# Anony-CFFM/CFFM

Measured on AMD Instinct MI355X. Metric: training examples/sec, frappe 10-field dim32; embedding-gather %HBM roofline, higher is better.
Workload: dtype f32; 1 GPU; frappe shape: synthetic libfm, 10 fields, 5382 features, inner/outer dim 32, batch 256 per GPU, selu, Adagrad lr 0.05, square_loss (README.md:28); global_batch=256, id_distribution=uniform, tables=replicated, parallelism=single

## Files before the change

### cffm_amd/csrc/common.hpp

```cpp
#pragma once
#include <hip/hip_runtime.h>
#include <stdint.h>

#include "../../include/cffm_hip.h"

#define CFFM_WAVE 64

#ifdef CFFM_PHASE_TIMERS
static __device__ unsigned long long cffm_phase_times[16];
static __device__ unsigned long long cffm_wg_times[2 * 1024];
static __device__ unsigned long long cffm_bwd_times[48];
#define PHASE_MARKB(i, wg) do { if ((wg) == 7 && threadIdx.x == 0) cffm_bwd_times[i] = wall_clock64(); } while (0)
#define PHASE_MARK(i) do { if (blockIdx.x == 7 && threadIdx.x == 0) cffm_phase_times[i] = wall_clock64(); } while (0)
#define PHASE_MARK2(i) do {} while (0)
#define PHASE_MARK3(i) do { if (CL && blockIdx.x == 7 && threadIdx.x == 0) cffm_phase_times[8 + (i)] = wall_clock64(); } while (0)
#else
#define PHASE_MARK(i) do {} while (0)
#define PHASE_MARK2(i) do {} while (0)
#define PHASE_MARK3(i) do {} while (0)
#define PHASE_MARKB(i, wg) do {} while (0)
#endif

typedef float f32x4 __attribute__((ext_vector_type(4)));
__device__ __forceinline__ int fused_c_off(int l, int c0, int c1, int D, int Pp) {
// ... 180 lines not shown
static inline int conv_slabs(const cffm_shape_t* s, int32_t B, int l) {
    const int64_t S = s->D >> (l + 1);
    if (bwd_fused01_ok(s, B)) {
        if (l <= 1) return 256;
        const int64_t n = ((int64_t)B * S * S + CFFM_TOP_SLAB_ROWS - 1) / CFFM_TOP_SLAB_ROWS;
        return n < 1 ? 1 : (int)n;
    }
    if (bwd_top_ok(s, B) && l >= bwd_top_first_layer(s)) {
        if (!top_wgrad_deferred(s, B)) return 256;
        const int64_t n = ((int64_t)B * S * S + 63) / 64;
        return n < 1 ? 1 : (n > 256 ? 256 : (int)n);
    }
    return conv_slabs_plain(s, B, l);
}

static inline void make_slab_plan(const cffm_shape_t* s, int32_t B, const cffm_theta_layout_t& tl, SlabPlan* p) {
    int n = 0;
    int64_t base = 0;
    auto add = [&](int64_t off, int64_t end, int nslab) {
        p->r[n].off = off; p->r[n].len = end - off; p->r[n].base = base; p->r[n].nslab = nslab;
        base += (end - off) * nslab;
        return n++;
    };
    const int64_t convs = tl.live > 0 ? tl.conv_w[0] : tl.d1_w;
    p->head_front = add(0, tl.inner_cw, small_slabs(B));
    p->inner = add(tl.inner_cw, convs, small_slabs(B));
    p->conv0 = n;
    for (int l = 0; l < tl.live; ++l)
        add(tl.conv_w[l], l + 1 < tl.live ? tl.conv_w[l + 1] : tl.d1_w, conv_slabs(s, B, l));
    p->head_back = add(tl.d1_w, tl.n, small_slabs(B));
    p->n = n;
    p->total = base;
}

__device__ __forceinline__ float head_dout(int loss, float out, float y, float invB, float L) {
    switch (loss) {
        case CFFM_LOSS_SQUARE_RMSE: return (out - y) * invB / L;
        case CFFM_LOSS_MSE: return 2.f * (out - y) * invB;
        case CFFM_LOSS_MAE: return (out > y ? 1.f : (out < y ? -1.f : 0.f)) * invB;
        case CFFM_LOSS_SQUARE_L2: return out - y;
        case CFFM_LOSS_HYBRID:
            return 0.5f * (out - y) - 0.5f * invB * (y / (out + 1e-7f) - (1.f - y) / (1.f - out + 1e-7f));
        default: {
            const float s = out;
            return -(y / (s + 1e-7f) - (1.f - y) / (1.f - s + 1e-7f)) * invB * s * (1.f - s);
        }
    }
}

#define CFFM_SELU_SCALE 1.0507009873554804934193349852946f
#define CFFM_SELU_SCALE_ALPHA 1.7580993408473768599402175208123f

__device__ __forceinline__ float act_f(float x, int act) {
    switch (act) {
        case CFFM_ACT_RELU: return fmaxf(x, 0.f);
        case CFFM_ACT_PRELU: return fmaxf(x, 0.f) + 0.25f * (-fmaxf(-x, 0.f));
        case CFFM_ACT_ELU: return x < 0.f ? expf(x) - 1.f : x;
        case CFFM_ACT_SELU: return x < 0.f ? CFFM_SELU_SCALE_ALPHA * (expf(x) - 1.f) : CFFM_SELU_SCALE * x;
        default: return x * (0.5f * (1.f + erff(x * 0.70710678118654752440f)));
    }
}

__device__ __forceinline__ float act_grad_f(float x, int act) {
    switch (act) {
        case CFFM_ACT_RELU: return x > 0.f ? 1.f : 0.f;
        case CFFM_ACT_PRELU: return x > 0.f ? 1.f : (x < 0.f ? 0.25f : 0.f);
        case CFFM_ACT_ELU: return x < 0.f ? expf(x) : 1.f;
        case CFFM_ACT_SELU: return x < 0.f ? CFFM_SELU_SCALE_ALPHA * expf(x) : CFFM_SELU_SCALE;
        default: {
            float cdf = 0.5f * (1.f + erff(x * 0.70710678118654752440f));
            float pdf = expf(-0.5f * x * x) * 0.39894228040143267794f;
            return cdf + x * pdf;
        }
    }
}

__device__ __forceinline__ float act_pos(float c, int act) {
    switch (act) {
        case CFFM_ACT_SELU: return CFFM_SELU_SCALE * c;
        case CFFM_ACT_GELU: return c * (0.5f * (1.f + erff(c * 0.70710678118654752440f)));
        default: return c;
    }
}

__device__ __forceinline__ float act_relu_grad(float c, int act) {
    return c > 0.f ? act_grad_f(c, act) : 0.f;
}

__device__ __forceinline__ void lds_barrier() {
    __builtin_amdgcn_fence(__ATOMIC_RELEASE, "workgroup", "local");
    __builtin_amdgcn_s_barrier();
    __builtin_amdgcn_fence(__ATOMIC_ACQUIRE, "workgroup", "local");
}

template <int CTRL, int ROW_MASK>
__device__ __forceinline__ float dpp_mov(float v, float identity) {
    return __builtin_bit_cast(float, __builtin_amdgcn_update_dpp(__builtin_bit_cast(int, identity), __builtin_bit_cast(int, v),
                                                                 CTRL, ROW_MASK, 0xf, false));
}
__device__ __forceinline__ float wave_sum(float v) {
    v += dpp_mov<0xB1, 0xf>(v, 0.f);
    v += dpp_mov<0x4E, 0xf>(v, 0.f);
    v += dpp_mov<0x141, 0xf>(v, 0.f);
    v += dpp_mov<0x140, 0xf>(v, 0.f);
    v += dpp_mov<0x142, 0xa>(v, 0.f);
    v += dpp_mov<0x143, 0xc>(v, 0.f);
    return __builtin_bit_cast(float, __builtin_amdgcn_readlane(__builtin_bit_cast(int, v), 63));
}
__device__ __forceinline__ float wave_max(float v) {
    const float ninf = -INFINITY;
    v = fmaxf(v, dpp_mov<0xB1, 0xf>(v, ninf));
    v = fmaxf(v, dpp_mov<0x4E, 0xf>(v, ninf));
    v = fmaxf(v, dpp_mov<0x141, 0xf>(v, ninf));
    v = fmaxf(v, dpp_mov<0x140, 0xf>(v, ninf));
    v = fmaxf(v, dpp_mov<0x142, 0xa>(v, ninf));
    v = fmaxf(v, dpp_mov<0x143, 0xc>(v, ninf));
    return __builtin_bit_cast(float, __builtin_amdgcn_readlane(__builtin_bit_cast(int, v), 63));
}

template <bool SIXTEEN>
__device__ __forceinline__ float row_group_sum(float v) {
    v += dpp_mov<0xB1, 0xf>(v, 0.f);
    v += dpp_mov<0x4E, 0xf>(v, 0.f);
    v += dpp_mov<0x141, 0xf>(v, 0.f);
    if (SIXTEEN) v += dpp_mov<0x140, 0xf>(v, 0.f);
    return v;
}

template <int NTH = 0>
__device__ __forceinline__ float block_sum(float v, float* red) {
    v = wave_sum(v);
    const int w = threadIdx.x >> 6, nw = NTH ? NTH >> 6 : (int)blockDim.x >> 6;
    __syncthreads();
    if ((threadIdx.x & 63) == 0 && (NTH == 0 || w < nw)) red[w] = v;
    __syncthreads();
    float t = 0.f;
    for (int i = 0; i < nw; ++i) t += red[i];
    return t;
}

template <int NTH = 0>
__device__ __forceinline__ void build_pair_lut(uint32_t* lut, int F, int Pp) {
    const int nth = NTH ? NTH : (int)blockDim.x;
    for (int i = threadIdx.x; i < F; i += nth) {
        int base = i * (2 * F - i - 1) / 2;
        for (int j = i + 1; j < F; ++j) lut[base + j - i - 1] = (uint32_t)i | ((uint32_t)j << 16);
    }
    const int P = F * (F - 1) / 2;
    for (int p = P + threadIdx.x; p < Pp; p += nth) lut[p] = 0u;
}

__device__ __forceinline__ int fast_div(int n, float inv_d) { return (int)(((float)n + 0.5f) * inv_d); }

__device__ __forceinline__ f32x4 mfma16(float a, float b, f32x4 c) {
    return __builtin_amdgcn_mfma_f32_16x16x4f32(a, b, c, 0, 0, 0);
}


template <int N, int NTH>
struct ParkFilter {
    float4 w[N];
    float4* dst;
    int n4;
    __device__ __forceinline__ void fetch(const float4* src, float4* dst_, int n4_) {
        dst = dst_; n4 = src != nullptr ? n4_ : 0;
#pragma unroll
        for (int ii = 0; ii < N; ++ii) {
            const int i = threadIdx.x + NTH * ii;
            w[ii] = i < n4 ? src[i] : make_float4(0.f, 0.f, 0.f, 0.f);
        }
    }
    __device__ __forceinline__ void operator()() const {
#pragma unroll
        for (int ii = 0; ii < N; ++ii) {
            const int i = threadIdx.x + NTH * ii;
            if (i < n4) dst[i] = w[ii];
        }
    }
};

template <int U, int NTH, class T, class Load, class Use>
__device__ __forceinline__ void loads_first(int tid, int n, Load&& load, Use&& use) {
    for (int e0 = tid; e0 < n; e0 += U * NTH) {
        T v[U];
#pragma unroll
        for (int u = 0; u < U; ++u) {
            const int e = e0 + u * NTH;
            if (e < n) v[u] = load(e);
        }
#pragma unroll
        for (int u = 0; u < U; ++u) {
            const int e = e0 + u * NTH;
            if (e < n) use(e, v[u]);
        }
    }
}
```

### cffm_amd/csrc/conv.hip

```cpp
#include <cstdlib>
#include <cstring>

#include "internal.hpp"

#include <type_traits>

#include <stdlib.h>
#include "inner_body.hpp"
#include "head_body.hpp"
#include "sort_body.hpp"

#define KSTEP 32
#define WG_KM 64

__device__ __forceinline__ int64_t xcd_tile(int64_t per_xcd) {
    const int64_t id = blockIdx.x;
    return (id & 7) * per_xcd + (id >> 3);
}
__host__ __device__ static inline int64_t xcd_per(int64_t tiles) { return (tiles + 7) / 8; }

struct RowPos { int b, y, x; };
__device__ __forceinline__ RowPos row_pos(int64_t m, int lgSo) {
    RowPos p;
    const int So = 1 << lgSo;
// ... 1549 lines not shown
    unsigned long long* keys_sorted;
    int live, n_rows, id_bits, B;
    int rank_keys;
    int c0_off, c1_off;
    int early_off, es_off;
};


__device__ __forceinline__ unsigned rank_key_id(int raw, int M) { return min((unsigned)raw, (unsigned)M); }
template <int NW, int F_ = 0>
__device__ __forceinline__ void rank_keys_body(const int32_t* __restrict__ ids, int n, int b, int F_rt, int M,
                                               unsigned long long* __restrict__ out, char* smem) {
    constexpr int MAXF = F_ ? F_ : RANK_MAXF;
    const int F = F_ ? F_ : F_rt;
    float* cnt = reinterpret_cast<float*>(smem);
    const int tid = threadIdx.x, lane = tid & 63, wave = tid >> 6;
    unsigned long long mine[MAXF];
#pragma unroll
    for (int f = 0; f < MAXF; ++f) {
        const int slot = b * F + (f < F ? f : 0);
        mine[f] = f < F ? (((unsigned long long)rank_key_id(ids[slot], M) << 32) | (unsigned)slot) : 0ull;
    }
    int c[MAXF];
#pragma unroll
    for (int f = 0; f < MAXF; ++f) c[f] = 0;
    constexpr int GRP = 8;
    for (int j0 = tid; j0 < n; j0 += 64 * NW * GRP) {
        unsigned idj[GRP];
#pragma unroll
        for (int u = 0; u < GRP; ++u) {
            const int j = j0 + 64 * NW * u;
            idj[u] = rank_key_id(ids[j < n ? j : n - 1], M);
        }
#pragma unroll
        for (int u = 0; u < GRP; ++u) {
            const int j = j0 + 64 * NW * u;
            const unsigned long long kj = j < n ? (((unsigned long long)idj[u] << 32) | (unsigned)j) : ~0ull;
#pragma unroll
            for (int f = 0; f < MAXF; ++f) c[f] += kj < mine[f] ? 1 : 0;
        }
    }
#pragma unroll
    for (int f = 0; f < MAXF; ++f) {
        const float t = wave_sum((float)c[f]);
        if (lane == 0) cnt[wave * RANK_MAXF + f] = t;
    }
    __syncthreads();
    if (tid < F) {
        float c = cnt[tid];
#pragma unroll
        for (int w = 1; w < NW; ++w) c += cnt[w * RANK_MAXF + tid];
        const int rank = (int)c;
        const int slot = b * F + tid;
        out[rank] = ((unsigned long long)rank_key_id(ids[slot], M) << 32) | (unsigned)slot;
    }
    __syncthreads();
}

template <int N> using IntC = std::integral_constant<int, N>;
#define CV(x) decltype(x)::value
template <int L0, int L1, class Fn>
__device__ __forceinline__ void static_for(Fn&& fn) {
    if constexpr (L0 < L1) { fn(IntC<L0>()); static_for<L0 + 1, L1>(fn); }
}

template <int NT, int G, int ACT, int LGSO = -1, int GT = G>
__device__ __forceinline__ void fused_layer_fwd(const ConvArgs& ca, int b, char* smem, const float* inL, float* outL) {
    const int lgSo = LGSO >= 0 ? LGSO : ca.lgSo;
    const int64_t rows = 1ll << (2 * lgSo), m_lo = (int64_t)b * rows, m_hi = m_lo + rows;
    if (rows >= 64) {
        for (int64_t m0 = m_lo; m0 < m_hi; m0 += 64) {
            if (m0 > m_lo) lds_barrier();
            conv_fwd_taps_body<NT, 4 / G, false, G, ACT, LGSO, GT>(ca, m0, m_hi, smem, inL, outL, m_lo);
        }
    } else if (rows >= 32) {
        conv_fwd_taps_body<NT, (G >= 2 ? 1 : 2), false, G, ACT, LGSO, GT>(ca, m_lo, m_hi, smem, inL, outL, m_lo);
    } else {
        conv_fwd_taps_body<NT, 1, false, G, ACT, LGSO, GT>(ca, m_lo, m_hi, smem, inL, outL, m_lo);
    }
}

static constexpr int fwd_all_layer_groups(int G, int lgSo) { return (G > 2 && lgSo <= 1) ? 2 : G; }

template <int NT, int NW, int ACT = -1, int F_ = 0, int K_ = 0, int D_ = 0>
__global__ __launch_bounds__(64 * NW) void fwd_all_kernel(FwdAllArgs fa) {
    constexpr int G = NW / 4, PP = NT * 16;
    constexpr bool CS = F_ != 0;
    constexpr FwdAllLds PL = fwd_all_lds_plan(CS ? F_ : 2, CS ? K_ : 4, CS ? D_ : 4, PP, NW);
    constexpr int NTS = CS ? 512 : 0;
    static_assert(!CS || 64 * NW >= NTS, "the workgroup holds the threads that sum inner_out");
    static_assert(!CS || (F_ * (F_ - 1) / 2 + 15) / 16 * 16 == PP, "NT is the column tile count of F_ fields");
    static_assert(!CS || (PL.c0_off >= 0 && PL.early_fits), "the compiled shape keeps its activations in LDS and gathers early");
    extern __shared__ __attribute__((aligned(16))) char smem[];
    const int c0_off = CS ? PL.c0_off : fa.c0_off, c1_off = CS ? PL.c1_off : fa.c1_off, es_off = CS ? PL.es_off : fa.es_off;
    const int D = CS ? D_ : fa.inner.g.D;
    int live = fa.live;
    if (CS) { live = -1; for (int d = D_; d > 1; d >>= 1) ++live; }
    auto CL = [&](int l) -> float* {
        return c0_off >= 0 ? reinterpret_cast<float*>(smem + fused_c_off(l, c0_off, c1_off, D, PP)) : nullptr;
    };
    const bool lds_act = c0_off >= 0;
#ifdef CFFM_PHASE_TIMERS
    if (threadIdx.x == 0) cffm_wg_times[2 * blockIdx.x] = wall_clock64();
#endif
    auto example = [&](int b) __attribute__((always_inline)) {
        ParkFilter<(4 * PP * PP / 4 + 64 * NW - 1) / (64 * NW), 64 * NW> park;
        const bool early = fa.early_off > 0;
        park.fetch(early ? reinterpret_cast<const float4*>(fa.conv[0].W) : nullptr, reinterpret_cast<float4*>(smem), 4 * PP * PP / 4);
        char* smem_i = smem + (CS ? (early ? PL.t_off : 0) : fa.early_off);
        if (fa.rank_keys) rank_keys_body<NW, F_>(fa.ids, fa.n_rows, b, fa.inner.g.F, fa.inner.g.M, fa.keys_sorted, smem_i);
        PHASE_MARK(0);
        inner_fwd_body<ACT, decltype(park), F_, K_, D_, NTS>(fa.inner, b, smem_i, early ? reinterpret_cast<float*>(smem + es_off) : nullptr,
                                                             D + 1, park);
        if (lds_act) lds_barrier(); else __syncthreads();
        PHASE_MARK(1);
        conv0_fact_fwd_body<NT, NW, F_, D_>(fa.conv[0], b, smem, CL(0), early);
        if constexpr (CS) {
            static_for<1, PL.live>([&](auto lc) __attribute__((always_inline)) {
                constexpr int l = CV(lc), LGSO = PL.lgS0 - l;
                lds_barrier();
                PHASE_MARK(1 + l);
                fused_layer_fwd<NT, fwd_all_layer_groups(G, LGSO), ACT, LGSO, G>(fa.conv[l], b, smem, CL(l - 1), CL(l));
            });
        } else {
            for (int l = 1; l < live; ++l) {
                if (lds_act) lds_barrier(); else __syncthreads();
                PHASE_MARK(1 + l);
                fused_layer_fwd<NT, G, ACT>(fa.conv[l], b, smem, CL(l - 1), CL(l));
            }
        }
        if (lds_act) lds_barrier(); else __syncthreads();
        PHASE_MARK(1 + live);
        head_fwd_body<NW, ACT, false, F_, D_>(fa.head, b, smem, lds_act, c0_off, c1_off);
        PHASE_MARK(2 + live);
    };
    if constexpr (CS) {
        static_assert(!CS || 4096 / (CS ? F_ : 1) <= 2 * 256, "two passes over a grid of 256 workgroups cover every accepted B");
        if ((int)blockIdx.x < fa.B) example((int)blockIdx.x);
        if (const int b = blockIdx.x + gridDim.x; b < fa.B) {
            __syncthreads();
            example(b);
        }
    } else {
        for (int b = blockIdx.x; b < fa.B; b += gridDim.x) {
            if (b != (int)blockIdx.x) __syncthreads();
            example(b);
        }
    }
#ifdef CFFM_PHASE_TIMERS
    if (threadIdx.x == 0) cffm_wg_times[2 * blockIdx.x + 1] = wall_clock64();
#endif
}

template <int NT, int F_, int D_, int NW, bool ONE = false>
__device__ __forceinline__ void conv0_fact_bwd_body(const DgradArgs& a, float* __restrict__ slabW, float* __restrict__ slabB,
                                                    int64_t slab_stride, char* smem, int wg, int nwg) {
    constexpr int PP = NT * 16, S = 16, NTH = 64 * NW, XQ = 16 / NW;
    const int F = F_ ? F_ : a.F, D = D_ ? D_ : a.D, Dp = D + 1, P = F_ ? F_ * (F_ - 1) / 2 : a.P, F2 = 2 * F;
    const int TP = S * PP + 16;
    float* Wl = reinterpret_cast<float*>(smem);
    float* T = Wl + 4 * PP * PP;
    float* part = T + 2 * F * TP;
    float* dEi = part + NW * 16 * 32;
    float* dEj = dEi + 32 * 16;
    float* bred = dEj + 32 * 16;
    float* rs = bred + NW * PP;
    float* Es = rs + 2 * F;
    const int tid = threadIdx.x, lane = tid & 63, wave = tid >> 6, r = lane & 15, kk = lane >> 4;
    float* sw = slabW + (int64_t)wg * slab_stride;
    float* sb = slabB + (int64_t)wg * slab_stride;
    PHASE_MARKB(12, wg);
    {
        ParkFilter<(4 * PP * PP / 4 + NTH - 1) / NTH, NTH> park;
        park.fetch(reinterpret_cast<const float4*>(a.W), reinterpret_cast<float4*>(Wl), 4 * PP * PP / 4);
        park();
        for (int e = tid; e < 4 * (PP - P) * PP; e += NTH) {
            const int tap = e / ((PP - P) * PP), o = e - tap * ((PP - P) * PP);
            sw[(tap * PP + P) * PP + o] = 0.f;
        }
    }
    bool first = true;
    float bacc[NT];
#pragma unroll
    for (int nt = 0; nt < NT; ++nt) bacc[nt] = 0.f;

    for (int b = wg; b < a.B; b += nwg) {
        __syncthreads();
        {
            const float* e = a.Cprev + (int64_t)b * F * D;
            const float invD = 1.f / (float)D;
            loads_first<2, NTH, float>(tid, F * D, [&](int i) { return e[i]; }, [&](int i, float v) {
                const int f = fast_div(i, invD), d = i - f * D;
                Es[f * Dp + d] = v;
            });
        }
        __syncthreads();
        const float* dCb = a.dC + (int64_t)b * S * S * PP;
        PHASE_MARKB(13, wg);
        for (int u = wave; u < 2 * (F - 1); u += NW) {
            const int i = u % (F - 1), dh = u / (F - 1);
            const int nj = F - 1 - i, K = 2 * nj, base = i * (2 * F - i - 1) / 2;
            f32x4 acc[NT];
#pragma unroll
            for (int nt = 0; nt < NT; ++nt) acc[nt] = (f32x4){0.f, 0.f, 0.f, 0.f};
            for (int k0 = 0; k0 < K; k0 += 4) {
                const int k = k0 + kk;
                const bool ok = k < K;
                const int dw = (ok && k >= nj) ? 1 : 0, jj = ok ? k - dw * nj : 0;
                const float av = ok ? Es[(i + 1 + jj) * Dp + 2 * r + dw] : 0.f;
                const float* wr = Wl + ((dh * 2 + dw) * PP + base + jj) * PP + r;
#pragma unroll
                for (int nt = 0; nt < NT; ++nt) acc[nt] = mfma16(av, ok ? wr[nt * 16] : 0.f, acc[nt]);
            }
            float* tp = T + (dh * F + i) * TP + r;
#pragma unroll
            for (int nt = 0; nt < NT; ++nt)
#pragma unroll
                for (int j = 0; j < 4; ++j) tp[(kk * 4 + j) * PP + nt * 16] = acc[nt][j];
        }
        for (int e = tid; e < 2 * S * PP; e += NTH) {
            const int dh = e / (S * PP), o = e - dh * (S * PP);
            T[(dh * F + F - 1) * TP + o] = 0.f;
        }
        __syncthreads();
        PHASE_MARKB(14, wg);
        {
            f32x4 acc[2] = {(f32x4){0.f, 0.f, 0.f, 0.f}, (f32x4){0.f, 0.f, 0.f, 0.f}};
            float4 av[XQ][NT];
#pragma unroll
            for (int q4 = 0; q4 < XQ; ++q4)
#pragma unroll
                for (int h = 0; h < NT; ++h)
                    av[q4][h] = *reinterpret_cast<const float4*>(dCb + ((int64_t)r * S + wave + NW * q4) * PP + 16 * h + 4 * kk);
#pragma unroll
            for (int q4 = 0; q4 < XQ; ++q4) {
                const int x = wave + NW * q4;
#pragma unroll
                for (int h = 0; h < NT; ++h) {
                    float4 bv[2];
#pragma unroll
                    for (int ct = 0; ct < 2; ++ct) {
                        const int n = ct * 16 + r;
                        bv[ct] = n < F2 ? *reinterpret_cast<const float4*>(T + n * TP + x * PP + 16 * h + 4 * kk)
                                        : make_float4(0.f, 0.f, 0.f, 0.f);
                    }
#pragma unroll
                    for (int ct = 0; ct < 2; ++ct) {
                        acc[ct] = mfma16(av[q4][h].x, bv[ct].x, acc[ct]);
                        acc[ct] = mfma16(av[q4][h].y, bv[ct].y, acc[ct]);
                        acc[ct] = mfma16(av[q4][h].z, bv[ct].z, acc[ct]);
                        acc[ct] = mfma16(av[q4][h].w, bv[ct].w, acc[ct]);
                    }
                }
            }
#pragma unroll
            for (int ct = 0; ct < 2; ++ct)
#pragma unroll
                for (int j = 0; j < 4; ++j) part[(wave * 16 + kk * 4 + j) * 32 + ct * 16 + r] = acc[ct][j];
        }
        __syncthreads();
        for (int e = tid; e < 16 * 32; e += NTH) {
            float v = part[e];
#pragma unroll
            for (int w = 1; w < NW; ++w) v += part[512 * w + e];
            dEi[(e & 31) * 16 + (e >> 5)] = v;
        }
        __syncthreads();
        PHASE_MARKB(15, wg);
        {
            float av[2][4];
#pragma unroll
            for (int rt = 0; rt < 2; ++rt)
#pragma unroll
                for (int s4 = 0; s4 < 4; ++s4) {
                    const int m = rt * 16 + r, dh = m >= F ? 1 : 0, i = m - dh * F;
                    av[rt][s4] = m < F2 ? Es[i * Dp + 2 * (4 * s4 + kk) + dh] : 0.f;
                }
#pragma unroll
            for (int q4 = 0; q4 < XQ; ++q4) {
                const int x = wave + NW * q4;
                float bv[4][NT];
#pragma unroll
                for (int s4 = 0; s4 < 4; ++s4)
#pragma unroll
                    for (int nt = 0; nt < NT; ++nt) bv[s4][nt] = dCb[((int64_t)(4 * s4 + kk) * S + x) * PP + nt * 16 + r];
                f32x4 acc[2][NT];
#pragma unroll
                for (int rt = 0; rt < 2; ++rt)
#pragma unroll
                    for (int nt = 0; nt < NT; ++nt) acc[rt][nt] = (f32x4){0.f, 0.f, 0.f, 0.f};
#pragma unroll
                for (int s4 = 0; s4 < 4; ++s4)
#pragma unroll
                    for (int nt = 0; nt < NT; ++nt) {
                        bacc[nt] += bv[s4][nt];
#pragma unroll
                        for (int rt = 0; rt < 2; ++rt) acc[rt][nt] = mfma16(av[rt][s4], bv[s4][nt], acc[rt][nt]);
                    }
#pragma unroll
                for (int rt = 0; rt < 2; ++rt)
#pragma unroll
                    for (int nt = 0; nt < NT; ++nt)
#pragma unroll
                        for (int j = 0; j < 4; ++j) {
                            const int m = rt * 16 + kk * 4 + j;
                            if (m < F2) T[m * TP + x * PP + nt * 16 + r] = acc[rt][nt][j];
                        }
            }
        }
        __syncthreads();
        PHASE_MARKB(16, wg);
        {
            int ucount = 0;
            for (int dh = 0; dh < 2; ++dh)
                for (int i = 0; i < F - 1; ++i) {
                    const int nj = F - 1 - i, K = 2 * nj, base = i * (2 * F - i - 1) / 2;
                    for (int rt = 0; rt * 16 < K; ++rt, ++ucount) {
                        if ((ucount & (NW - 1)) != wave) continue;
                        const int m = rt * 16 + r;
                        const bool okm = m < K;
                        const int dw = (okm && m >= nj) ? 1 : 0, jj = okm ? m - dw * nj : 0;
                        f32x4 acc[NT];
#pragma unroll
                        for (int nt = 0; nt < NT; ++nt) acc[nt] = (f32x4){0.f, 0.f, 0.f, 0.f};
#pragma unroll
                        for (int s4 = 0; s4 < 4; ++s4) {
                            const int x = 4 * s4 + kk;
                            const float avv = okm ? Es[(i + 1 + jj) * Dp + 2 * x + dw] : 0.f;
                            const float* tb = T + (dh * F + i) * TP + x * PP + r;
#pragma unroll
                            for (int nt = 0; nt < NT; ++nt) acc[nt] = mfma16(avv, tb[nt * 16], acc[nt]);
                        }
#pragma unroll
                        for (int j = 0; j < 4; ++j) {
                            const int mm = rt * 16 + kk * 4 + j;
                            if (mm < K) {
                                const int dw2 = mm >= nj ? 1 : 0, jj2 = mm - dw2 * nj;
                                float* dst = sw + ((dh * 2 + dw2) * PP + base + jj2) * PP + r;
#pragma unroll
                                for (int nt = 0; nt < NT; ++nt) dst[nt * 16] = first ? acc[nt][j] : dst[nt * 16] + acc[nt][j];
                            }
                        }
                    }
                }
        }
        PHASE_MARKB(17, wg);
        {
            f32x4 acc[2] = {(f32x4){0.f, 0.f, 0.f, 0.f}, (f32x4){0.f, 0.f, 0.f, 0.f}};
            int ud = 0;
            for (int i = 0; i < F - 1; ++i) ud += 2 * ((2 * (F - 1 - i) + 15) / 16);
            for (int u = (wave + NW - ud % NW) % NW; u < 2 * (F - 1); u += NW) {
                const int i = u % (F - 1), dh = u / (F - 1), base = i * (2 * F - i - 1) / 2;
                const float* ta = T + (dh * F + i) * TP + r * PP + 4 * kk;
                const float* wrow[2];
                bool okc[2];
#pragma unroll
                for (int ct = 0; ct < 2; ++ct) {
                    const int n = ct * 16 + r, dw = n >= F ? 1 : 0, j = n - dw * F;
                    okc[ct] = n < F2 && j > i;
                    wrow[ct] = Wl + ((dh * 2 + dw) * PP + base + (okc[ct] ? j - i - 1 : 0)) * PP + 4 * kk;
                }
#pragma unroll
                for (int h = 0; h < NT; ++h) {
                    const float4 av = *reinterpret_cast<const float4*>(ta + 16 * h);
#pragma unroll
                    for (int ct = 0; ct < 2; ++ct) {
                        const float4 bv = okc[ct] ? *reinterpret_cast<const float4*>(wrow[ct] + 16 * h) : make_float4(0.f, 0.f, 0.f, 0.f);
                        acc[ct] = mfma16(av.x, bv.x, acc[ct]);
                        acc[ct] = mfma16(av.y, bv.y, acc[ct]);
                        acc[ct] = mfma16(av.z, bv.z, acc[ct]);
                        acc[ct] = mfma16(av.w, bv.w, acc[ct]);
                    }
                }
            }
#pragma unroll
            for (int ct = 0; ct < 2; ++ct)
#pragma unroll
                for (int j = 0; j < 4; ++j) part[(wave * 16 + kk * 4 + j) * 32 + ct * 16 + r] = acc[ct][j];
        }
        PHASE_MARKB(18, wg);
        if (tid < 2 * F) {
            const int f = tid % F;
            float sacc = 0.f;
            if (tid < F) { for (int h = 0; h < D; ++h) sacc += Es[f * Dp + h]; }
            else { for (int h = 0; h < D; ++h) sacc += Es[f * Dp + h] * a.dt1[(int64_t)b * a.t1w + h]; }
            rs[tid] = sacc;
        }
        __syncthreads();
        for (int e = tid; e < 16 * 32; e += NTH) {
            float v = part[e];
#pragma unroll
            for (int w = 1; w < NW; ++w) v += part[512 * w + e];
            dEj[(e & 31) * 16 + (e >> 5)] = v;
        }
        __syncthreads();
        PHASE_MARKB(19, wg);
        for (int e = tid; e < F * D; e += NTH) {
            const int f = e / D, h = e - f * D, lo = h & 1, hh = h >> 1;
            float R = 0.f, Q = 0.f;
            for (int j = f + 1; j < F; ++j) R += rs[j];
            for (int i = 0; i < f; ++i) Q += rs[F + i];
            a.dprev[(int64_t)b * F * D + e] = (dEi[(lo * F + f) * 16 + hh] + dEj[(lo * F + f) * 16 + hh])
                                              + a.dt1[(int64_t)b * a.t1w + h] * R + Q;
        }
        first = false;
        if constexpr (ONE) break;
    }
    PHASE_MARKB(20, wg);
    __syncthreads();
#pragma unroll
    for (int nt = 0; nt < NT; ++nt) {
        float v = bacc[nt];
        v += __shfl_xor(v, 16, 64);
        v += __shfl_xor(v, 32, 64);
        if (kk == 0) bred[wave * PP + nt * 16 + r] = v;
    }
    __syncthreads();
    if (tid < PP) {
        float v = bred[tid];
#pragma unroll
        for (int w = 1; w < NW; ++w) v += bred[w * PP + tid];
        sb[tid] = v;
    }
    if (first) {
        for (int e = tid; e < 4 * PP * PP; e += NTH) sw[e] = 0.f;
    }
    PHASE_MARKB(25, wg);
}

template <int NT, int F_, int D_, int NW>
__global__ __launch_bounds__(64 * NW) void conv0_fact_bwd_kernel(DgradArgs a, float* __restrict__ slabW,
                                                              float* __restrict__ slabB, int64_t slab_stride) {
    extern __shared__ __attribute__((aligned(16))) char smem[];
    conv0_fact_bwd_body<NT, F_, D_, NW>(a, slabW, slabB, slab_stride, smem, blockIdx.x, gridDim.x);
}

template <int NT, int RM, bool L0, int HALVES, int ACTC = -1>
__device__ __forceinline__ void dgrad_taps_body(const DgradArgs& a, int wg, char* smem, int64_t m_lo = 0, int64_t m_end = -1,
                                                int tiles = 1, int tid_in = -1) {
    const int act = ACTC >= 0 ? ACTC : a.act;
    constexpr int PP = NT * 16, BM = 16 * RM, NTH = 256 * HALVES, NCOPY = 4 * HALVES;
    uint32_t* lut = reinterpret_cast<uint32_t*>(smem);
    float* Es = reinterpret_cast<float*>(lut + PP);
    const int tid = tid_in >= 0 ? tid_in : (int)threadIdx.x, lane = tid & 63, wid = tid >> 6, tap = wid & 3, half = wid >> 2, r = lane & 15, kk = lane >> 4;
    const int So = 1 << a.lgSo, Sin = 2 * So, P = a.P, Dp = a.D + 1, S2 = So * So, dh = tap >> 1, dw = tap & 1;
    const int rows_per_wg = L0 ? (S2 > BM ? S2 : BM) : BM * tiles;
    const int n_ex = L0 ? rows_per_wg / S2 : 0;
    const int mtiles = rows_per_wg / BM;
    const int64_t Mend = m_end < 0 ? a.Mtot : m_end;
    const int64_t wg_m0 = m_lo + (int64_t)wg * rows_per_wg;
    const int b0 = (int)(wg_m0 >> (2 * a.lgSo));
    const int exsz = a.F * Dp;
    const bool fast = L0 && RM == 4 && a.lgSo >= 4 && a.lgSo <= 6;
    float* rs = Es + n_ex * exsz;
    float* scratch = rs + 2 * n_ex * a.F;
    float* dEw = scratch + wid * (n_ex * exsz);
    float* Ti = scratch;
    float* Tj = Ti + 4 * PP * So;

    float4 bw[NT][NT];
#pragma unroll
    for (int nt = 0; nt < NT; ++nt) {
        const float* src = a.W + (int64_t)(tap * PP + nt * 16 + r) * PP + 4 * kk;
#pragma unroll
        for (int h = 0; h < NT; ++h) bw[nt][h] = *reinterpret_cast<const float4*>(src + 16 * h);
    }
    uint32_t ij[NT];
    if (L0) {
        build_pair_lut(lut, a.F, PP);
        stage_examples(Es, a.Cprev, b0, n_ex, a.B, a.F, a.D, Dp);
        if (!fast)
            for (int e = tid; e < NCOPY * n_ex * exsz; e += NTH) scratch[e] = 0.f;
        __syncthreads();
#pragma unroll
        for (int nt = 0; nt < NT; ++nt) ij[nt] = lut[nt * 16 + r];
    }
    float accj[RM][NT][4];
#pragma unroll
    for (int rm = 0; rm < RM; ++rm)
#pragma unroll
        for (int nt = 0; nt < NT; ++nt)
#pragma unroll
            for (int j = 0; j < 4; ++j) accj[rm][nt][j] = 0.f;

    const int mt_per = (mtiles + HALVES - 1) / HALVES;
    const int mt_lo = half * mt_per, mt_hi = min(mtiles, mt_lo + mt_per);
    const int tpy = So >> 4;
    for (int mt = mt_lo; mt < mt_hi; ++mt) {
        const int64_t m0 = wg_m0 + (int64_t)mt * BM;
        float4 av[RM][NT];
#pragma unroll
        for (int rm = 0; rm < RM; ++rm) {
            int64_t m = m0 + rm * 16 + r;
            if (m >= Mend) m = Mend - 1;
#pragma unroll
            for (int h = 0; h < NT; ++h) av[rm][h] = *reinterpret_cast<const float4*>(a.dC + m * PP + 16 * h + 4 * kk);
        }
        float cpre[L0 ? 1 : RM][L0 ? 1 : NT][4], dpre[L0 ? 1 : RM][4];
        int64_t ppos[L0 ? 1 : RM][4];
        if (!L0) {
#pragma unroll
            for (int rm = 0; rm < RM; ++rm)
#pragma unroll
                for (int j = 0; j < 4; ++j) {
                    int64_t m = m0 + rm * 16 + kk * 4 + j;
                    if (m >= Mend) m = Mend - 1;
                    const RowPos rp = row_pos(m, a.lgSo);
                    ppos[rm][j] = (((int64_t)rp.b * Sin + 2 * rp.y + dh) * Sin + 2 * rp.x + dw) * PP + r;
                    dpre[rm][j] = a.dt1[(int64_t)rp.b * a.t1w + a.t1off + 2 * rp.y + dh];
#pragma unroll
                    for (int nt = 0; nt < NT; ++nt) cpre[rm][nt][j] = a.Cprev[ppos[rm][j] + nt * 16];
                }
        }
        f32x4 acc[RM][NT];
#pragma unroll
        for (int rm = 0; rm < RM; ++rm)
#pragma unroll
            for (int nt = 0; nt < NT; ++nt) acc[rm][nt] = (f32x4){0.f, 0.f, 0.f, 0.f};
#pragma unroll
        for (int h = 0; h < NT; ++h)
#pragma unroll
            for (int t = 0; t < 4; ++t)
#pragma unroll
                for (int rm = 0; rm < RM; ++rm) {
                    const float x = t == 0 ? av[rm][h].x : t == 1 ? av[rm][h].y : t == 2 ? av[rm][h].z : av[rm][h].w;
#pragma unroll
                    for (int nt = 0; nt < NT; ++nt) {
                        const float y = t == 0 ? bw[nt][h].x : t == 1 ? bw[nt][h].y : t == 2 ? bw[nt][h].z : bw[nt][h].w;
                        acc[rm][nt] = mfma16(x, y, acc[rm][nt]);
                    }
                }
        float si_run[NT];
#pragma unroll
        for (int nt = 0; nt < NT; ++nt) si_run[nt] = 0.f;
#pragma unroll
        for (int rm = 0; rm < RM; ++rm) {
            const int64_t mrow = m0 + rm * 16 + kk * 4;
            const RowPos rq = row_pos(mrow < Mend ? mrow : Mend - 1, a.lgSo);
#pragma unroll
            for (int nt = 0; nt < NT; ++nt) {
                const int p = nt * 16 + r;
                if (!L0) {
#pragma unroll
                    for (int j = 0; j < 4; ++j) {
                        if (mrow + j < Mend) {
                            const float g = acc[rm][nt][j] + dpre[L0 ? 0 : rm][j];
                            a.dprev[ppos[L0 ? 0 : rm][j] + nt * 16] = g * act_relu_grad(cpre[L0 ? 0 : rm][L0 ? 0 : nt][j], act);
                        }
                    }
                } else {
                    const int fi = ij[nt] & 0xffff, fj = ij[nt] >> 16;
                    const bool pv = p < P;
                    if (fast) {
                        const float ei = Es[fi * Dp + 2 * rq.y + dh];
                        float si = 0.f;
#pragma unroll
// ... 1977 lines not shown
```

Before: 3.099 million examples/s.

## Prefetch conv0 backward operands into registers ahead of the filter park

Restructures the conv0 factorized backward body so each example's embedding slice, dC tiles and dt1 row are loaded into registers at the top of the iteration. In the single-example path this happens before the filter is parked to shared memory, so global-memory latency overlaps the filter staging. dt1 is cached in a shared row (reusing the bred buffer) instead of being re-read from global memory. Several shared-memory index products switch to 24-bit multiplies. The cost is higher register pressure from holding dC fragments across phases, which could reduce occupancy. Reusing bred as drow is safe only if bred is not written inside the loop.

Measured after the change: 3.123 million examples/s (median of 6 runs). About the same (+0.8%).

```diff
diff --git a/cffm_amd/csrc/common.hpp b/cffm_amd/csrc/common.hpp
--- a/cffm_amd/csrc/common.hpp
+++ b/cffm_amd/csrc/common.hpp
@@ -356,6 +356,8 @@
 
 __device__ __forceinline__ int fast_div(int n, float inv_d) { return (int)(((float)n + 0.5f) * inv_d); }
 
+__device__ __forceinline__ int mul24(int a, int b) { return (int)__umul24((unsigned)a, (unsigned)b); }
+
 __device__ __forceinline__ f32x4 mfma16(float a, float b, f32x4 c) {
     return __builtin_amdgcn_mfma_f32_16x16x4f32(a, b, c, 0, 0, 0);
 }
diff --git a/cffm_amd/csrc/conv.hip b/cffm_amd/csrc/conv.hip
--- a/cffm_amd/csrc/conv.hip
+++ b/cffm_amd/csrc/conv.hip
@@ -1725,6 +1725,24 @@
 #endif
 }
 
+template <int NT, int NW>
+struct Conv0Head {
+    static constexpr int PP = NT * 16, NTH = 64 * NW;
+    static constexpr int EU = (11 * 32 + NTH - 1) / NTH;
+    ParkFilter<(4 * PP * PP / 4 + NTH - 1) / NTH, NTH> park;
+    float ev[EU], dv;
+    __device__ __forceinline__ void fetch_filter(const DgradArgs& a, char* smem) {
+        park.fetch(reinterpret_cast<const float4*>(a.W), reinterpret_cast<float4*>(smem), 4 * PP * PP / 4);
+    }
+    __device__ __forceinline__ void fetch_example(const DgradArgs& a, int b, int F, int D) {
+        const int tid = threadIdx.x;
+        const float* e = a.Cprev + (int64_t)b * F * D;
+#pragma unroll
+        for (int u = 0; u < EU; ++u) ev[u] = tid + u * NTH < F * D ? e[tid + u * NTH] : 0.f;
+        dv = tid < D ? a.dt1[(int64_t)b * a.t1w + tid] : 0.f;
+    }
+};
+
 template <int NT, int F_, int D_, int NW, bool ONE = false>
 __device__ __forceinline__ void conv0_fact_bwd_body(const DgradArgs& a, float* __restrict__ slabW, float* __restrict__ slabB,
                                                     int64_t slab_stride, char* smem, int wg, int nwg) {
@@ -1742,33 +1760,56 @@
     const int tid = threadIdx.x, lane = tid & 63, wave = tid >> 6, r = lane & 15, kk = lane >> 4;
     float* sw = slabW + (int64_t)wg * slab_stride;
     float* sb = slabB + (int64_t)wg * slab_stride;
+    float* drow = bred;
     PHASE_MARKB(12, wg);
-    {
-        ParkFilter<(4 * PP * PP / 4 + NTH - 1) / NTH, NTH> park;
-        park.fetch(reinterpret_cast<const float4*>(a.W), reinterpret_cast<float4*>(Wl), 4 * PP * PP / 4);
-        park();
+    Conv0Head<NT, NW> q;
+    q.fetch_filter(a, smem);
+    auto filter_in = [&]() {
+        q.park();
         for (int e = tid; e < 4 * (PP - P) * PP; e += NTH) {
             const int tap = e / ((PP - P) * PP), o = e - tap * ((PP - P) * PP);
             sw[(tap * PP + P) * PP + o] = 0.f;
         }
-    }
+    };
+    if constexpr (!ONE) filter_in();
     bool first = true;
     float bacc[NT];
 #pragma unroll
     for (int nt = 0; nt < NT; ++nt) bacc[nt] = 0.f;
 
+    constexpr int EU = Conv0Head<NT, NW>::EU;
     for (int b = wg; b < a.B; b += nwg) {
+        if constexpr (!ONE) __syncthreads();
+        const float* dCb = a.dC + (int64_t)b * S * S * PP;
+        float4 dca[XQ][NT];
+        float dcb[XQ][4][NT];
+        {
+            q.fetch_example(a, b, F, D);
+#pragma unroll
+            for (int q4 = 0; q4 < XQ; ++q4)
+#pragma unroll
+                for (int h = 0; h < NT; ++h)
+                    dca[q4][h] = *reinterpret_cast<const float4*>(dCb + ((int64_t)r * S + wave + NW * q4) * PP + 16 * h + 4 * kk);
+#pragma unroll
+            for (int q4 = 0; q4 < XQ; ++q4)
+#pragma unroll
+                for (int s4 = 0; s4 < 4; ++s4)
+#pragma unroll
+                    for (int nt = 0; nt < NT; ++nt)
+                        dcb[q4][s4][nt] = dCb[((int64_t)(4 * s4 + kk) * S + wave + NW * q4) * PP + nt * 16 + r];
+            if constexpr (ONE) filter_in();
+            const float invD = 1.f / (float)D;
+#pragma unroll
+            for (int u = 0; u < EU; ++u) {
+                const int i = tid + u * NTH;
+                if (i < F * D) {
+                    const int f = fast_div(i, invD), d = i - f * D;
+                    Es[f * Dp + d] = q.ev[u];
+                }
+            }
+            if (tid < D) drow[tid] = q.dv;
+        }
         __syncthreads();
-        {
-            const float* e = a.Cprev + (int64_t)b * F * D;
-            const float invD = 1.f / (float)D;
-            loads_first<2, NTH, float>(tid, F * D, [&](int i) { return e[i]; }, [&](int i, float v) {
-                const int f = fast_div(i, invD), d = i - f * D;
-                Es[f * Dp + d] = v;
-            });
-        }
-        __syncthreads();
-        const float* dCb = a.dC + (int64_t)b * S * S * PP;
         PHASE_MARKB(13, wg);
         for (int u = wave; u < 2 * (F - 1); u += NW) {
             const int i = u % (F - 1), dh = u / (F - 1);
@@ -1780,12 +1821,12 @@
                 const int k = k0 + kk;
                 const bool ok = k < K;
                 const int dw = (ok && k >= nj) ? 1 : 0, jj = ok ? k - dw * nj : 0;
-                const float av = ok ? Es[(i + 1 + jj) * Dp + 2 * r + dw] : 0.f;
-                const float* wr = Wl + ((dh * 2 + dw) * PP + base + jj) * PP + r;
+                const float av = ok ? Es[mul24(i + 1 + jj, Dp) + 2 * r + dw] : 0.f;
+                const float* wr = Wl + mul24((dh * 2 + dw) * PP + base + jj, PP) + r;
 #pragma unroll
                 for (int nt = 0; nt < NT; ++nt) acc[nt] = mfma16(av, ok ? wr[nt * 16] : 0.f, acc[nt]);
             }
-            float* tp = T + (dh * F + i) * TP + r;
+            float* tp = T + mul24(dh * F + i, TP) + r;
 #pragma unroll
             for (int nt = 0; nt < NT; ++nt)
 #pragma unroll
@@ -1799,12 +1840,6 @@
         PHASE_MARKB(14, wg);
         {
             f32x4 acc[2] = {(f32x4){0.f, 0.f, 0.f, 0.f}, (f32x4){0.f, 0.f, 0.f, 0.f}};
-            float4 av[XQ][NT];
-#pragma unroll
-            for (int q4 = 0; q4 < XQ; ++q4)
-#pragma unroll
-                for (int h = 0; h < NT; ++h)
-                    av[q4][h] = *reinterpret_cast<const float4*>(dCb + ((int64_t)r * S + wave + NW * q4) * PP + 16 * h + 4 * kk);
 #pragma unroll
             for (int q4 = 0; q4 < XQ; ++q4) {
                 const int x = wave + NW * q4;
@@ -1819,10 +1854,10 @@
                     }
 #pragma unroll
                     for (int ct = 0; ct < 2; ++ct) {
-                        acc[ct] = mfma16(av[q4][h].x, bv[ct].x, acc[ct]);
-                        acc[ct] = mfma16(av[q4][h].y, bv[ct].y, acc[ct]);
-                        acc[ct] = mfma16(av[q4][h].z, bv[ct].z, acc[ct]);
-                        acc[ct] = mfma16(av[q4][h].w, bv[ct].w, acc[ct]);
+                        acc[ct] = mfma16(dca[q4][h].x, bv[ct].x, acc[ct]);
+                        acc[ct] = mfma16(dca[q4][h].y, bv[ct].y, acc[ct]);
+                        acc[ct] = mfma16(dca[q4][h].z, bv[ct].z, acc[ct]);
+                        acc[ct] = mfma16(dca[q4][h].w, bv[ct].w, acc[ct]);
                     }
                 }
             }
@@ -1852,11 +1887,7 @@
 #pragma unroll
             for (int q4 = 0; q4 < XQ; ++q4) {
                 const int x = wave + NW * q4;
-                float bv[4][NT];
-#pragma unroll
-                for (int s4 = 0; s4 < 4; ++s4)
-#pragma unroll
-                    for (int nt = 0; nt < NT; ++nt) bv[s4][nt] = dCb[((int64_t)(4 * s4 + kk) * S + x) * PP + nt * 16 + r];
+                const auto& bv = dcb[q4];
                 f32x4 acc[2][NT];
 #pragma unroll
                 for (int rt = 0; rt < 2; ++rt)
@@ -1956,7 +1987,7 @@
             const int f = tid % F;
             float sacc = 0.f;
             if (tid < F) { for (int h = 0; h < D; ++h) sacc += Es[f * Dp + h]; }
-            else { for (int h = 0; h < D; ++h) sacc += Es[f * Dp + h] * a.dt1[(int64_t)b * a.t1w + h]; }
+            else { for (int h = 0; h < D; ++h) sacc += Es[f * Dp + h] * drow[h]; }
             rs[tid] = sacc;
         }
         __syncthreads();
@@ -1974,7 +2005,7 @@
             for (int j = f + 1; j < F; ++j) R += rs[j];
             for (int i = 0; i < f; ++i) Q += rs[F + i];
             a.dprev[(int64_t)b * F * D + e] = (dEi[(lo * F + f) * 16 + hh] + dEj[(lo * F + f) * 16 + hh])
-                                              + a.dt1[(int64_t)b * a.t1w + h] * R + Q;
+                                              + drow[h] * R + Q;
         }
         first = false;
         if constexpr (ONE) break;
```
